# ALIZE-Speaker-Recognition/LIA_RAL

Measured on AMD Instinct MI355X. Metric: Gframe-Gaussian evals/s (UBM EM pass: LLK + full-posterior statistics), higher is better.
Workload: dtype f64; 1 GPU; TrainWorld EM: 2048-Gaussian diag UBM, 60-dim float32 frames, 10000000 frames per GPU resident in HBM, 1 EM iteration per step; gaussians=2048, dim=60, frames_per_gpu=10000000, partitioning=frames sharded per rank, one RCCL all-reduce of 247810 doubles per step

## Files before the change

lia_ral_amd/csrc/devutil.h:

```cpp
#pragma once
#include <hip/hip_runtime.h>
#include <stdint.h>

typedef double d4 __attribute__((ext_vector_type(4)));

#define MFMA_F64(a, b, c) __builtin_amdgcn_mfma_f64_16x16x4f64((a), (b), (c), 0, 0, 0)

#define GMMIV_NEG_BIG (-1.0e300)
#define GMMIV_ZERO_LLK (-745.1332191019412)
#define GMMIV_PAD_LOGIT (-1.0e9)

__device__ __forceinline__ double gexp(double x)
{
    x = fmax(x, -750.0);
    const double n = __builtin_rint(x * 1.4426950408889634074);
    double r = __builtin_fma(n, -6.93147180369123816490e-01, x);
    r = __builtin_fma(n, -1.90821492927058770002e-10, r);
    double p = 1.6059043836821613e-10;
    p = __builtin_fma(p, r, 2.08767569878681e-09);
    p = __builtin_fma(p, r, 2.505210838544172e-08);
    p = __builtin_fma(p, r, 2.755731922398589e-07);
    p = __builtin_fma(p, r, 2.7557319223985893e-06);
    p = __builtin_fma(p, r, 2.48015873015873e-05);
    p = __builtin_fma(p, r, 1.984126984126984e-04);
// ... 153 lines not shown
    GMMIV_ARGMAX_STEP(0x121)
#undef GMMIV_ARGMAX_STEP
    const double v0 = __hiloint2double(__builtin_amdgcn_readlane(__double2hiint(v), 0), __builtin_amdgcn_readlane(__double2loint(v), 0));
    const int c0 = __builtin_amdgcn_readlane(c, 0);
    double wv = v0;
    int wc = c0;
#pragma unroll
    for (int r = 1; r < 4; ++r) {
        const double ov = __hiloint2double(__builtin_amdgcn_readlane(__double2hiint(v), 16 * r), __builtin_amdgcn_readlane(__double2loint(v), 16 * r));
        const int oc = __builtin_amdgcn_readlane(c, 16 * r);
        if (ov > wv || (ov == wv && oc < wc)) { wv = ov; wc = oc; }
    }
    v = wv;
    c = wc;
}

__device__ __forceinline__ double dpp_f64_0x128(double v) { return __hiloint2double(dpp_i32<0x128>(__double2hiint(v)), dpp_i32<0x128>(__double2loint(v))); }
__device__ __forceinline__ double dpp_f64_0x124(double v) { return __hiloint2double(dpp_i32<0x124>(__double2hiint(v)), dpp_i32<0x124>(__double2loint(v))); }
__device__ __forceinline__ double dpp_f64_0x122(double v) { return __hiloint2double(dpp_i32<0x122>(__double2hiint(v)), dpp_i32<0x122>(__double2loint(v))); }
__device__ __forceinline__ double dpp_f64_0x121(double v) { return __hiloint2double(dpp_i32<0x121>(__double2hiint(v)), dpp_i32<0x121>(__double2loint(v))); }
__device__ __forceinline__ double readlane_f64u(double v, int l)
{
    return __hiloint2double(__builtin_amdgcn_readlane(__double2hiint(v), l), __builtin_amdgcn_readlane(__double2loint(v), l));
}
__device__ __forceinline__ double wave_sum_f64_dpp(double v)
{
    v += dpp_f64_0x128(v); v += dpp_f64_0x124(v); v += dpp_f64_0x122(v); v += dpp_f64_0x121(v);
    return (readlane_f64u(v, 0) + readlane_f64u(v, 16)) + (readlane_f64u(v, 32) + readlane_f64u(v, 48));
}
__device__ __forceinline__ double half_sum_f64_dpp(double v, bool hi)
{
    v += dpp_f64_0x128(v); v += dpp_f64_0x124(v); v += dpp_f64_0x122(v); v += dpp_f64_0x121(v);
    const double a = readlane_f64u(v, 0) + readlane_f64u(v, 16), b = readlane_f64u(v, 32) + readlane_f64u(v, 48);
    return hi ? b : a;
}
__device__ __forceinline__ double half_max_f64_dpp(double v, bool hi)
{
    v = fmax(v, dpp_f64_0x128(v)); v = fmax(v, dpp_f64_0x124(v)); v = fmax(v, dpp_f64_0x122(v)); v = fmax(v, dpp_f64_0x121(v));
    const double a = fmax(readlane_f64u(v, 0), readlane_f64u(v, 16)), b = fmax(readlane_f64u(v, 32), readlane_f64u(v, 48));
    return hi ? b : a;
}
__device__ __forceinline__ double half_min_f64_dpp(double v, bool hi)
{
    v = fmin(v, dpp_f64_0x128(v)); v = fmin(v, dpp_f64_0x124(v)); v = fmin(v, dpp_f64_0x122(v)); v = fmin(v, dpp_f64_0x121(v));
    const double a = fmin(readlane_f64u(v, 0), readlane_f64u(v, 16)), b = fmin(readlane_f64u(v, 32), readlane_f64u(v, 48));
    return hi ? b : a;
}
__device__ __forceinline__ double wave_max_f64_dpp(double v)
{
    v = fmax(v, dpp_f64_0x128(v)); v = fmax(v, dpp_f64_0x124(v)); v = fmax(v, dpp_f64_0x122(v)); v = fmax(v, dpp_f64_0x121(v));
    return fmax(fmax(readlane_f64u(v, 0), readlane_f64u(v, 16)), fmax(readlane_f64u(v, 32), readlane_f64u(v, 48)));
}
__device__ __forceinline__ double wave_min_f64_dpp(double v)
{
    v = fmin(v, dpp_f64_0x128(v)); v = fmin(v, dpp_f64_0x124(v)); v = fmin(v, dpp_f64_0x122(v)); v = fmin(v, dpp_f64_0x121(v));
    return fmin(fmin(readlane_f64u(v, 0), readlane_f64u(v, 16)), fmin(readlane_f64u(v, 32), readlane_f64u(v, 48)));
}

__device__ __forceinline__ double shfl_xor_f64(double v, int mask)
{
    int lo = __double2loint(v), hi = __double2hiint(v);
    lo = __shfl_xor(lo, mask, 64);
    hi = __shfl_xor(hi, mask, 64);
    return __hiloint2double(hi, lo);
}

__device__ __forceinline__ double wave_sum_f64(double v)
{
#pragma unroll
    for (int o = 32; o > 0; o >>= 1) v += shfl_xor_f64(v, o);
    return v;
}
__device__ __forceinline__ double wave_max_f64(double v)
{
#pragma unroll
    for (int o = 32; o > 0; o >>= 1) v = fmax(v, shfl_xor_f64(v, o));
    return v;
}

__device__ __forceinline__ int xswz(int t) { return ((t << 1) ^ ((t & 1) << 4)) & 31; }

__device__ __forceinline__ int xrot(int t) { return ((t & 1) << 4) + (((t >> 1) & 7) << 1); }

__device__ __forceinline__ int div_by_magic(unsigned e, unsigned magic) { return magic ? (int)__umulhi(e, magic) : (int)e; }
static inline unsigned gmmiv_div_magic(int D) { return D == 1 ? 0u : (unsigned)((1ULL << 32) / (unsigned)D + 1); }

#define GMMIV_UNUSABLE_BOUND 1e18
#define GMMIV_UNUSABLE_READ_AS 1e10
#ifndef GMMIV_FEAT_SANE_OFF
__device__ __forceinline__ float feat_sane(float v) { return __builtin_fabsf(v) <= (float)GMMIV_UNUSABLE_BOUND ? v : (float)GMMIV_UNUSABLE_READ_AS; }
__device__ __forceinline__ double feat_sane(double v) { return __builtin_fabs(v) <= GMMIV_UNUSABLE_BOUND ? v : GMMIV_UNUSABLE_READ_AS; }
#else
__device__ __forceinline__ float feat_sane(float v) { return v; }
__device__ __forceinline__ double feat_sane(double v) { return v; }
#endif
template <typename T> struct feat_load;
template <> struct feat_load<float> {
    static __device__ __forceinline__ double get(const void *p, long i) { return (double)feat_sane(((const float *)p)[i]); }
    static __device__ __forceinline__ double raw(const void *p, long i) { return (double)((const float *)p)[i]; }
};
template <> struct feat_load<double> {
    static __device__ __forceinline__ double get(const void *p, long i) { return feat_sane(((const double *)p)[i]); }
    static __device__ __forceinline__ double raw(const void *p, long i) { return ((const double *)p)[i]; }
};
```

lia_ral_amd/csrc/gmm_kernels.hip:

```cpp
#include <atomic>
#include "devutil.h"
#include "lds_attr.h"
#include "gmm_kernels.h"

typedef double d2v __attribute__((ext_vector_type(2)));

__global__ void k_gmm_const(int C, int Cp, int D, const double *__restrict__ w,
                            const double *__restrict__ mean, const double *__restrict__ iv,
                            double *__restrict__ a, double *__restrict__ logwcst)
{
    int c = blockIdx.x * blockDim.x + threadIdx.x;
    if (c >= Cp) return;
    if (c >= C) { a[c] = GMMIV_NEG_BIG; logwcst[c] = GMMIV_NEG_BIG; return; }
    double sl = 0.0, sm = 0.0;
    for (int d = 0; d < D; ++d) {
        double v = iv[(size_t)c * D + d], m = mean[(size_t)c * D + d];
        sl += log(v);
        sm += m * m * v;
    }
    double lw = (w[c] > 0.0) ? log(w[c]) : GMMIV_NEG_BIG;
    double lc = lw - 0.5 * D * 1.8378770664093454836 + 0.5 * sl;
    lc = fmax(lc, GMMIV_NEG_BIG);
    logwcst[c] = lc;
    a[c] = fmax(lc - 0.5 * sm, GMMIV_NEG_BIG);
// ... 229 lines not shown
                    gexp_tab_reduce(acc[1][h][r], k1[r], r1);
                    acc[0][h][r] = r0;
                    acc[1][h][r] = r1;
                    const int km = k0[r] > k1[r] ? k0[r] : k1[r];
                    nm[r] = km >> GEXP_TAB_BITS;
                    grow |= nm[r] - E[h][r] >= 64;
                }
                if (__builtin_amdgcn_ballot_w64(grow) != 0) {
#pragma unroll
                    for (int r = 0; r < 4; ++r) {
                        nm[r] = row_max_i32(nm[r]);
                        if (nm[r] - E[h][r] >= 64) {
                            int sh = E[h][r] - nm[r];
                            sh = sh < -2000 ? -2000 : sh;
                            sacc[h][r] = __builtin_ldexp(sacc[h][r], sh);
                            E[h][r] = nm[r];
                        }
                    }
                }
#pragma unroll
                for (int r = 0; r < 4; ++r) {
                    const double e0 = gexp_tab_finish(k0[r], acc[0][h][r], E[h][r], etab);
                    const double e1 = gexp_tab_finish(k1[r], acc[1][h][r], E[h][r], etab);
                    sacc[h][r] += (hit0[r] ? 0.0 : e0) + (hit1[r] ? 0.0 : e1);
                }
            }
            return;
        }
        if (WZ || (MODE == 0 && K1_PLAIN_SHARED)) {
            int nm[2][4], k0[2][4], k1[2][4];
            bool grow = false;
#pragma unroll
            for (int h = 0; h < 2; ++h)
#pragma unroll
                for (int r = 0; r < 4; ++r) {
                    double r0, r1;
                    gexp_tab_reduce(acc[0][h][r], k0[h][r], r0);
                    gexp_tab_reduce(acc[1][h][r], k1[h][r], r1);
                    acc[0][h][r] = r0;
                    acc[1][h][r] = r1;
                    const int km = k0[h][r] > k1[h][r] ? k0[h][r] : k1[h][r];
                    nm[h][r] = km >> GEXP_TAB_BITS;
                    grow |= nm[h][r] - E[h][r] >= 64;
                }
            if (__builtin_amdgcn_ballot_w64(grow) != 0) {
#pragma unroll
                for (int h = 0; h < 2; ++h)
#pragma unroll
                    for (int r = 0; r < 4; ++r) {
                        if (!(K1_ABL & 8)) nm[h][r] = row_max_i32(nm[h][r]);
                        if (nm[h][r] - E[h][r] >= 64) {
                            int sh = E[h][r] - nm[h][r];
                            sh = sh < -2000 ? -2000 : sh;
                            sacc[h][r] = __builtin_ldexp(sacc[h][r], sh);
                            E[h][r] = nm[h][r];
                        }
                    }
            }
#pragma unroll
            for (int h = 0; h < 2; ++h)
#pragma unroll
                for (int r = 0; r < 4; ++r) {
                    const double e0 = gexp_tab_finish(k0[h][r], acc[0][h][r], E[h][r], (K1_ABL & 2) ? etab - (k0[h][r] & (GEXP_TAB_N - 1)) : etab);
                    const double e1 = gexp_tab_finish(k1[h][r], acc[1][h][r], E[h][r], (K1_ABL & 2) ? etab - (k1[h][r] & (GEXP_TAB_N - 1)) : etab);
                    sacc[h][r] += e0 + e1;
                    acc[0][h][r] = e0;
                    acc[1][h][r] = e1;
                }
            if (!WZ) return;
            if (!late) asm volatile("s_waitcnt vmcnt(0)" ::: "memory");
            double *zw = zbuf + ((((size_t)(te * GT)) * nfb + (tb >> 4)) * 64 + lane) * 4;
            if (K1_ABL & 4) {
#pragma unroll
                for (int g = 0; g < GT; ++g)
#pragma unroll
                    for (int h = 0; h < 2; ++h) asm volatile("" ::"v"(acc[g][h]));
                return;
            }
#pragma unroll
            for (int g = 0; g < GT; ++g)
#pragma unroll
                for (int h = 0; h < 2; ++h) __builtin_nontemporal_store(acc[g][h], (d4 *)(zw + ((size_t)g * nfb + h) * 256));
            if (i16 == 0 && !(K1_ABL & 32)) {
                int *ew = eit + (size_t)te * (nfb * 16) + tb + q;
#pragma unroll
                for (int h = 0; h < 2; ++h)
#pragma unroll
                    for (int r = 0; r < 4; ++r) ew[h * 16 + 4 * r] = E[h][r];
            }
            return;
        }
        int nm[2][4];
        bool grow = false;
#pragma unroll
        for (int h = 0; h < 2; ++h)
#pragma unroll
            for (int r = 0; r < 4; ++r) {
                nm[h][r] = gexp_tab_exponent(fmax(acc[0][h][r], acc[1][h][r]));
                grow |= nm[h][r] - E[h][r] >= 64;
            }
        if (__builtin_amdgcn_ballot_w64(grow) != 0) {
#pragma unroll
            for (int h = 0; h < 2; ++h)
#pragma unroll
                for (int r = 0; r < 4; ++r)
                    if (nm[h][r] - E[h][r] >= 64) {
                        int sh = E[h][r] - nm[h][r];
                        sh = sh < -2000 ? -2000 : sh;
                        sacc[h][r] = __builtin_ldexp(sacc[h][r], sh);
                        E[h][r] = nm[h][r];
                    }
        }
        unsigned need = 0;
#pragma unroll
        for (int h = 0; h < 2; ++h)
#pragma unroll
            for (int r = 0; r < 4; ++r) {
                nref[h][r] = nm[h][r] > nref[h][r] ? nm[h][r] : nref[h][r];
                need |= (__builtin_amdgcn_ballot_w64(nm[h][r] > nref[h][r] - 57) != 0 ? 1u : 0u) << (h * 4 + r);
            }
        if (__builtin_popcount(need) > 3) {
#pragma unroll
            for (int h = 0; h < 2; ++h)
#pragma unroll
                for (int r = 0; r < 4; ++r)
                    sacc[h][r] += gexp_tab_scaled(acc[0][h][r], E[h][r], etab) + gexp_tab_scaled(acc[1][h][r], E[h][r], etab);
        } else if (need) {
#pragma unroll
            for (int h = 0; h < 2; ++h)
#pragma unroll
                for (int r = 0; r < 4; ++r)
                    if (need & (1u << (h * 4 + r)))
                        sacc[h][r] += gexp_tab_scaled(acc[0][h][r], E[h][r], etab) + gexp_tab_scaled(acc[1][h][r], E[h][r], etab);
        }
    };
    stage(buf0, 0);
    __syncthreads();
    auto step = [&](int tl, bool staged, bool is_late, bool first) __attribute__((always_inline)) {
        double *cur = (tl & 1) ? buf1 : buf0;
        double *nxt = (tl & 1) ? buf0 : buf1;
        if (staged && (TC || dbg < 2) && !(K1_ABL & 16)) stage(nxt, tl + 1);
        if (!is_late) {
            mfma_phase(cur);
            epi_phase(tl);
        } else {
            if (!first) epi_phase(tl - 1);
            mfma_phase(cur);
        }
        if (WZ) {
            if (is_late) asm volatile("s_waitcnt vmcnt(0)" ::: "memory");
            if (!(K1_ABL & 16)) asm volatile("s_waitcnt lgkmcnt(0)\n\ts_barrier" ::: "memory");
        } else {
            __syncthreads();
        }
    };
    if (!late) {
        for (int tl = 0; tl + 1 < ntiles; ++tl) step(tl, true, false, false);
        if (ntiles > 0) step(ntiles - 1, false, false, false);
    } else {
        if (ntiles > 1) step(0, true, true, true);
        for (int tl = 1; tl + 1 < ntiles; ++tl) step(tl, true, true, false);
        if (ntiles > 0) step(ntiles - 1, false, true, ntiles == 1);
    }
    if (late && ntiles > 0) epi_phase(ntiles - 1);
#pragma unroll
    for (int h = 0; h < 2; ++h)
#pragma unroll
        for (int r = 0; r < 4; ++r) {
            int Em = E[h][r];
#pragma unroll
            for (int o = 1; o < 16; o <<= 1) { const int oe = __shfl_xor(Em, o, 64); Em = oe > Em ? oe : Em; }
// ... 1220 lines not shown
```

lia_ral_amd/csrc/stats_z.hip:

```cpp
#include <atomic>
#include "devutil.h"
#include "lds_attr.h"
#include "gmm_kernels.h"

template <int KS, bool SQ, typename XT, bool PRUNE, int NW = 8, int TPW = 2, int FT = 64, int ZD = 2>
__global__ __launch_bounds__(NW * 64, (TPW == 1 ? 4 : 2)) void k_stats_z(const void *__restrict__ x, long ldx, int D, int C, int nct,
                                                    const double *__restrict__ zbuf, long nfb, const int *__restrict__ eit,
                                                    const double *__restrict__ inv, const int *__restrict__ efin, double scale,
                                                    const long *__restrict__ seg_begin, int nseg, int ngrp,
                                                    double *__restrict__ out0, double *__restrict__ out1, int mode, int accum,
                                                    unsigned magicD, double prune_arg)
{
    constexpr int Dp = 4 * KS;
    constexpr int RL = ((Dp + 2 + 31) / 32) * 32;
    constexpr int JT = RL / 16;
    constexpr int NT = NW * 64;
    constexpr int BPT = FT / 16;
    constexpr int NLD = (FT * Dp + NT - 1) / NT;
    constexpr int RLp = RL + 32;
    constexpr int PF = TPW > 2 ? TPW / 2 : 1;
    extern __shared__ __attribute__((aligned(16))) char smem[];
    double *buf0 = (double *)smem;
    double *buf1 = buf0 + FT * RLp;

    const int b = blockIdx.x;
    const int seg_lo = b & 7;
    const int rest = b >> 3;
    const int grp = rest % ngrp;
    const int seg = (rest / ngrp) * 8 + seg_lo;
    if (seg >= nseg) return;

    const int tid = threadIdx.x, lane = tid & 63, wave = tid >> 6;
    const int i16 = lane & 15, q = lane >> 4;
    const int ct0 = (grp * NW + wave) * TPW;
    const bool active = ct0 < nct;

    const long f0 = seg_begin[seg], f1 = seg_begin[seg + 1];
    const long fa = f0 & ~15L;
    const int nblk = f1 > f0 ? (int)((f1 - fa + 15) >> 4) : 0;
    const int ntiles = (nblk + BPT - 1) / BPT;

    d4 S[TPW][JT], S2[TPW][SQ ? JT : 1];
#pragma unroll
    for (int t = 0; t < TPW; ++t) {
#pragma unroll
        for (int j = 0; j < JT; ++j) S[t][j] = (d4){0, 0, 0, 0};
#pragma unroll
        for (int j = 0; j < (SQ ? JT : 1); ++j) S2[t][j] = (d4){0, 0, 0, 0};
    }

    typedef double d2 __attribute__((ext_vector_type(2)));
    XT stg[NLD];
    double stg_inv = 0.0;
    int stg_ef = 0, stg_e[PF];
    const int npad = FT * (RL - D);
    constexpr bool PLAN_IN_REGS = TPW < 4;
    const bool contig = (ldx == D);
    auto plan_pk = [&](int i) -> unsigned {
        const int e = tid + NT * i;
        const int fr = div_by_magic((unsigned)e, magicD), d = e - fr * D;
        return fr < FT ? ((unsigned)fr << 16) | (unsigned)((fr * RLp + xrot(fr) + d) * 8) : 0xffff0000u;
    };
    auto plan_goff = [&](int i) -> unsigned {
        const int e = tid + NT * i;
        const int fr = div_by_magic((unsigned)e, magicD), d = e - fr * D;
        return fr < FT ? (contig ? (unsigned)e : (unsigned)(fr * (int)ldx + d)) : 0u;
    };
    unsigned pk_r[PLAN_IN_REGS ? NLD : 1], goff_r[PLAN_IN_REGS ? NLD : 1];
    if constexpr (PLAN_IN_REGS) {
#pragma unroll
        for (int i = 0; i < NLD; ++i) { pk_r[i] = plan_pk(i); goff_r[i] = plan_goff(i); }
    }
#define PK(i) (PLAN_IN_REGS ? pk_r[PLAN_IN_REGS ? (i) : 0] : plan_pk(i))
#define GOFF(i) (PLAN_IN_REGS ? goff_r[PLAN_IN_REGS ? (i) : 0] : plan_goff(i))
    double *ftile = buf1 + FT * RLp;
    const int *epair[PF];
#pragma unroll
    for (int p = 0; p < PF; ++p) epair[p] = eit + (size_t)(active ? (ct0 >> 1) + p : 0) * (nfb * 16) + fa;
    const int srow = lane & (FT - 1);
    auto issue_stage = [&](int tl) {
        const long fb = fa + (long)tl * FT;
        const long rem = f1 - fb;
        const unsigned lim = rem >= FT ? (unsigned)FT << 16 : (unsigned)rem << 16;
        const XT *xt = (const XT *)x + fb * ldx;
#pragma unroll
        for (int i = 0; i < NLD; ++i) {
            stg[i] = xt[PK(i) < lim ? GOFF(i) : 0u];
        }
        const long t = fb + srow < f1 ? fb + srow : f1 - 1;
        stg_inv = inv[t];
        stg_ef = efin[t];
#pragma unroll
        for (int p = 0; p < PF; ++p) stg_e[p] = epair[p][(long)tl * FT + srow];
    };
    auto finish_stage = [&](double *dst, int buf, int tl) {
        const long fb = fa + (long)tl * FT;
        const long rem = f1 - fb;
        const unsigned lim = rem >= FT ? (unsigned)FT << 16 : (unsigned)rem << 16;
#pragma unroll
        for (int i = 0; i < NLD; ++i)
        {
            const unsigned pki = PK(i);
            if (pki < ((unsigned)FT << 16)) *(double *)((char *)dst + (pki & 0xffffu)) = pki < lim ? (double)feat_sane(stg[i]) : 0.0;
        }
        if (lane < FT) {
            const long t = fb + lane;
#pragma unroll
            for (int p = 0; p < PF; ++p)
                ftile[((buf * NW + wave) * PF + p) * FT + lane] = (t >= f0 && t < f1) ? __builtin_ldexp(stg_inv * scale, stg_e[p] - stg_ef) : 0.0;
        }
    };
    for (int e = tid; e < 2 * npad; e += NT) {
        double *dst = e < npad ? buf0 : buf1;
        const int ee = e < npad ? e : e - npad;
        const int fr = ee / (RL - D), d = D + (ee - fr * (RL - D));
        dst[fr * RLp + xrot(fr) + d] = (d == Dp) ? 1.0 : 0.0;
    }

    const int offS = q * RLp + ((q & 1) << 4) + ((q >> 1) << 1) + i16;

    const double *zp0 = zbuf + ((((size_t)(active ? ct0 : 0)) * nfb + (fa >> 4)) * 64 + lane) * 4;
    const size_t ztile = (size_t)nfb * 256;
    static_assert((FT / 16) % ZD == 0, "the stream sets must divide the blocks of a tile");
    d2 zs[ZD][TPW][2];
#pragma unroll
    for (int b = 0; b < ZD; ++b)
#pragma unroll
        for (int t = 0; t < TPW; ++t) { zs[b][t][0] = (d2){0, 0}; zs[b][t][1] = zs[b][t][0]; }
    auto issue_z = [&](d2 (&z)[TPW][2], int n) {
#pragma unroll
        for (int t = 0; t < TPW; ++t) {
            const d2 *pz = (const d2 *)(zp0 + (size_t)t * ztile + (size_t)n * 256);
            z[t][0] = __builtin_nontemporal_load(pz);
            z[t][1] = __builtin_nontemporal_load(pz + 1);
        }
    };
    static_assert(TPW == 1 || TPW == 2 || TPW == 4, "operand list of PIN_Z");
#define PIN_Z(z)                                                                                              \
    do {                                                                                                      \
        if constexpr (TPW == 1) asm volatile("" : "+v"(z[0][0]), "+v"(z[0][1]));                             \
        else if constexpr (TPW == 2) asm volatile("" : "+v"(z[0][0]), "+v"(z[0][1]), "+v"(z[1][0]), "+v"(z[1][1])); \
        else asm volatile("" : "+v"(z[0][0]), "+v"(z[0][1]), "+v"(z[1][0]), "+v"(z[1][1]), "+v"(z[TPW / 2][0]),     \
                          "+v"(z[TPW / 2][1]), "+v"(z[TPW - 1][0]), "+v"(z[TPW - 1][1]));                      \
    } while (0)

    if (ntiles > 0) {
        issue_stage(0);
        if (active) {
#pragma unroll
            for (int b = 0; b + 1 < ZD; ++b) issue_z(zs[b], b < nblk ? b : nblk - 1);
        }
        finish_stage(buf0, 0, 0);
#pragma unroll
        for (int b = 0; b + 1 < ZD; ++b) PIN_Z(zs[b]);
    }
    __syncthreads();
    auto tile = [&](int tl, bool full) {
        const double *cur = (tl & 1) ? buf1 : buf0;
        double *nxt = (tl & 1) ? buf0 : buf1;
        const bool staged = full || tl + 1 < ntiles;
        if (staged) issue_stage(tl + 1);
        if (active) {
            const double *pS = cur + offS;
            const double *pF = ftile + ((tl & 1) * NW + wave) * PF * FT + q;
            auto block = [&](int fs, d2 (&zc)[TPW][2], d2 (&zn)[TPW][2]) {
                const int n = tl * BPT + fs;
                if (full) issue_z(zn, (ZD == 2 || n + ZD - 1 < nblk) ? n + ZD - 1 : nblk - 1);
                else if (n + ZD - 1 < nblk) issue_z(zn, n + ZD - 1);
#pragma unroll
                for (int r = 0; r < 4; ++r) {
                    double f[PF];
#pragma unroll
                    for (int p = 0; p < PF; ++p) f[p] = pF[p * FT + fs * 16 + 4 * r];
                    double gm[TPW];
                    bool keep = false;
#pragma unroll
                    for (int t = 0; t < TPW; ++t) { gm[t] = zc[t][r >> 1][r & 1] * f[PF > 1 ? t >> 1 : 0]; keep |= gm[t] > prune_arg; }
                    if (PRUNE && __builtin_amdgcn_ballot_w64(keep) == 0) continue;
#pragma unroll
                    for (int j = 0; j < JT; ++j) {
                        const double bv = pS[(fs * 16 + 4 * r) * RLp + 4 * r + 16 * j];
#pragma unroll
                        for (int t = 0; t < TPW; ++t) S[t][j] = MFMA_F64(gm[t], bv, S[t][j]);
                        if (SQ) {
                            const double b2 = bv * bv;
#pragma unroll
                            for (int t = 0; t < TPW; ++t) S2[t][j] = MFMA_F64(gm[t], b2, S2[t][j]);
                        }
                    }
                }
            };
            const int nb = nblk - tl * BPT;
            block(0, zs[0], zs[ZD - 1]);
            if (full || nb > 1) block(1, zs[1 % ZD], zs[0]);
            if (BPT > 2) {
                if (full || nb > 2) block(2, zs[2 % ZD], zs[1 % ZD]);
                if (full || nb > 3) block(3, zs[3 % ZD], zs[2 % ZD]);
            }
#pragma unroll
            for (int b = 0; b + 1 < ZD; ++b) PIN_Z(zs[b]);
        }
        if (staged) finish_stage(nxt, (tl + 1) & 1, tl + 1);
        __syncthreads();
    };
    for (int tl = 0; tl + 1 < ntiles; ++tl) tile(tl, true);
    if (ntiles > 0) tile(ntiles - 1, false);
#undef PIN_Z
#undef PK
#undef GOFF
    if (!active) return;
#pragma unroll
    for (int t = 0; t < TPW; ++t) {
        const int ct = ct0 + t;
        if (mode == 0) {
            const size_t Cp = (size_t)nct * 16;
            double *o = out0 + (size_t)seg * Cp * (2 * RL);
#pragma unroll
            for (int r = 0; r < 4; ++r) {
                const size_t c = (size_t)ct * 16 + q + 4 * r;
#pragma unroll
                for (int j = 0; j < JT; ++j) {
                    double *o1 = o + c * (2 * RL) + 16 * j + i16;
                    *o1 = (accum ? *o1 : 0.0) + S[t][j][r];
                    if (SQ) { double *o2 = o1 + RL; *o2 = (accum ? *o2 : 0.0) + S2[t][j][r]; }
                }
            }
        } else {
            double *N = out0 + (size_t)seg * C;
            double *F = out1 + (size_t)seg * C * D;
#pragma unroll
            for (int r = 0; r < 4; ++r) {
                const int c = ct * 16 + q + 4 * r;
                if (c >= C) continue;
#pragma unroll
                for (int j = 0; j < JT; ++j) {
                    const int col = 16 * j + i16;
                    if (col < D) F[(size_t)c * D + col] = S[t][j][r];
                    else if (col == Dp) N[c] = S[t][j][r];
                }
            }
        }
    }
}

#define HIPCHK(e)                                                         \
    do {                                                                  \
        hipError_t _e = (e);                                              \
        if (_e != hipSuccess) return (int)_e;                             \
    } while (0)

#define g_stats_z_waves (gmmiv_kopts_cur().z_waves)
#define g_stats_z_tv4 (gmmiv_kopts_cur().z_tv4)
#define g_stats_z_depth_em (gmmiv_kopts_cur().z_depth_em)
#define g_stats_z_depth_tv (gmmiv_kopts_cur().z_depth_tv)
int gmmk_stats_z_groups(int nct) { const int tpg = g_stats_z_waves == 4 ? 8 : 16; return (nct + tpg - 1) / tpg; }
int gmmk_stats_z_wg_per_cu(void) { return g_stats_z_waves == 4 ? 2 : 1; }

template <int KS, bool SQ, typename XT, bool PRUNE, int NW, int TPW, int FT, int ZD = 2>
static int launch_z(hipStream_t st, const void *x, long ldx, int D, int C, int nct, const double *zbuf, long nfb, const int *eit,
                    const double *inv, const int *efin, double scale, const long *seg_begin, int nseg, double *out0, double *out1,
                    int mode, int accum, double prune_thr)
{
    constexpr int RL = ((4 * KS + 2 + 31) / 32) * 32;
    constexpr int PF = TPW > 2 ? TPW / 2 : 1;
    const size_t lds = (size_t)2 * FT * (RL + 32) * sizeof(double) + (size_t)2 * NW * PF * FT * sizeof(double);
    HIPCHK((gmmiv_lds_attr<k_stats_z<KS, SQ, XT, PRUNE, NW, TPW, FT, ZD>>(lds)));
    const int ngrp = (nct + TPW * NW - 1) / (TPW * NW);
    const unsigned grid = (unsigned)(ngrp * 8 * ((nseg + 7) / 8));
    const unsigned magicD = gmmiv_div_magic(D);
    k_stats_z<KS, SQ, XT, PRUNE, NW, TPW, FT, ZD><<<grid, NW * 64, lds, st>>>(x, ldx, D, C, nct, zbuf, nfb, eit, inv, efin, scale, seg_begin, nseg, ngrp,
                                                              out0, out1, mode, accum, magicD, prune_thr);
    return (int)hipGetLastError();
}

#define ZARGS st, x, ldx, D, C, nct, zbuf, nfb, eit, inv, efin, scale, seg_begin, nseg, out0, out1, mode, accum, prune_thr
template <int KS, bool SQ, typename XT>
static int launch_z_p(hipStream_t st, const void *x, long ldx, int D, int C, int nct, const double *zbuf, long nfb, const int *eit,
                      const double *inv, const int *efin, double scale, const long *seg_begin, int nseg, double *out0, double *out1,
                      int mode, int accum, double prune_thr)
{
    if (prune_thr > 0.0) return launch_z<KS, SQ, XT, true, 8, 2, 64>(ZARGS);
    if (g_stats_z_waves == 4) return launch_z<KS, SQ, XT, false, 4, 2, 32>(ZARGS);
    if (g_stats_z_waves == 16) return launch_z<KS, SQ, XT, false, 16, 1, 64>(ZARGS);
    if constexpr (!SQ) {
        if (g_stats_z_depth_tv == 4) return launch_z<KS, SQ, XT, false, 8, 2, 64, 4>(ZARGS);
        if (g_stats_z_tv4 && nct % 4 == 0) return launch_z<KS, SQ, XT, false, 8, 4, 64>(ZARGS);
    } else if (g_stats_z_depth_em == 4) return launch_z<KS, SQ, XT, false, 8, 2, 64, 4>(ZARGS);
    return launch_z<KS, SQ, XT, false, 8, 2, 64>(ZARGS);
}

int gmmk_stats_z(hipStream_t st, int KS, int sq, int x_f64, const void *x, long ldx, int D, int C, int nct, const double *zbuf,
                 long nfb, const int *eit, const double *inv, const int *efin, double scale, const long *seg_begin, int nseg,
                 double *out0, double *out1, int mode, int accum, double prune_thr)
{
    if (nseg <= 0) return 0;
#define CASE(K)                                                                                      \
    case K:                                                                                          \
        if (sq) return x_f64 ? launch_z_p<K, true, double>(ZARGS) : launch_z_p<K, true, float>(ZARGS); \
        return x_f64 ? launch_z_p<K, false, double>(ZARGS) : launch_z_p<K, false, float>(ZARGS);
    switch (KS) {
        CASE(4) CASE(8) CASE(15)
    }
#undef CASE
    return -1;
}
```

lia_ral_amd/csrc/topc_z.hip:

```cpp
#include "devutil.h"
#include "gmm_kernels.h"

typedef double d2 __attribute__((ext_vector_type(2)));

template <typename XT>
__global__ __launch_bounds__(256, 2) void k_topc_from_z(const void *__restrict__ x, long n, long ldx, int D, int C, int nct,
                                                        const double *__restrict__ zbuf, long nfb, const int *__restrict__ eit,
                                                        const int *__restrict__ efin, const double *__restrict__ mean,
                                                        const double *__restrict__ iv, const double *__restrict__ lwc,
                                                        const double *__restrict__ w, int ctop, int complete, double lo, double hi,
                                                        int *__restrict__ idx_out, double *__restrict__ lk_out,
                                                        double *__restrict__ nontop_lk, double *__restrict__ nontop_llk,
                                                        double *__restrict__ nontop_w, double *__restrict__ llk_out, int *__restrict__ flag)
{
    __shared__ double xs[8][64 + 1];
    __shared__ int ord[4][64];
    __shared__ __attribute__((aligned(16))) double lmx[4][64];
    __shared__ double thx[4];
    const int tid = threadIdx.x, lane = tid & 63, wave = tid >> 6, i16 = lane & 15, qq = lane >> 4;
    const long fb = blockIdx.x >> 1;
    const int half = blockIdx.x & 1, q0 = wave;
    for (int e = tid; e < 8 * D; e += 256) {
        const int lf = e / D, d = e - lf * D;
        const long t = fb * 16 + (lf >> 1) + 4 * (2 * half + (lf & 1));
        xs[lf][d] = t < n ? feat_load<XT>::get(x, t * ldx + d) : 0.0;
    }
    long tj[2];
    int ef[2];
#pragma unroll
    for (int j = 0; j < 2; ++j) {
        tj[j] = fb * 16 + q0 + 4 * (2 * half + j);
        ef[j] = tj[j] < n ? efin[tj[j]] : 0;
    }
    double val[2][32];
#pragma unroll
    for (int h = 0; h < 2; ++h) {
        d2 e2[16];
        int e0[16], e1[16];
#pragma unroll
        for (int mm = 0; mm < 16; ++mm) {
            const int ct = 4 * (16 * h + mm) + qq, cc = ct < nct ? ct : nct - 1;
            e2[mm] = *(const d2 *)(zbuf + (((size_t)cc * nfb + fb) * 64 + 16 * q0 + i16) * 4 + 2 * half);
            const int *ep = eit + (size_t)(cc >> 1) * (nfb * 16) + fb * 16 + q0 + 8 * half;
            e0[mm] = ep[0];
            e1[mm] = ep[4];
        }
        asm volatile("" ::: "memory");
#pragma unroll
        for (int mm = 0; mm < 16; ++mm) {
            const int m = 16 * h + mm, ct = 4 * m + qq;
            const double a0 = __builtin_ldexp(e2[mm][0], e0[mm] - ef[0]), a1 = __builtin_ldexp(e2[mm][1], e1[mm] - ef[1]);
            val[0][m] = ct < nct ? a0 : -1.0;
            val[1][m] = ct < nct ? a1 : -1.0;
        }
    }
    __syncthreads();

    const double NINF = -__builtin_inf();
    const int K = ctop + 4 < C ? ctop + 4 : C;
#pragma unroll
    for (int j = 0; j < 2; ++j) {
        const long t = tj[j];
        if (t >= n) continue;
        const int lf = 2 * wave + j;
        double lm;
        {
            double t16[16];
#pragma unroll
            for (int i = 0; i < 16; ++i) t16[i] = fmax(val[j][i], val[j][i + 16]);
#pragma unroll
            for (int i = 0; i < 8; ++i) t16[i] = fmax(t16[i], t16[i + 8]);
#pragma unroll
            for (int i = 0; i < 4; ++i) t16[i] = fmax(t16[i], t16[i + 4]);
            lm = fmax(fmax(t16[0], t16[2]), fmax(t16[1], t16[3]));
        }
        lmx[wave][lane] = lm;
        __builtin_amdgcn_fence(__ATOMIC_RELEASE, "wavefront");
        __builtin_amdgcn_wave_barrier();
        __builtin_amdgcn_fence(__ATOMIC_ACQUIRE, "wavefront");
        int lrank = 0;
#pragma unroll
        for (int i = 0; i < 64; ++i) {
            const double o = lmx[wave][i];
            lrank += (o > lm || (o == lm && i < lane)) ? 1 : 0;
        }
        if (lrank == K - 1) thx[wave] = lm;
        __builtin_amdgcn_fence(__ATOMIC_RELEASE, "wavefront");
        __builtin_amdgcn_wave_barrier();
        __builtin_amdgcn_fence(__ATOMIC_ACQUIRE, "wavefront");
        double theta = thx[wave];
        __builtin_amdgcn_wave_barrier();
        if (!(theta > 0.0)) theta = 4.9e-324;
        int nc = 0;
#pragma unroll
        for (int m = 0; m < 32; ++m) {
            const bool hit = val[j][m] >= theta;
            const unsigned long long mask = __builtin_amdgcn_ballot_w64(hit);
            if (mask) {
                if (hit) {
                    const int pos = nc + __builtin_popcountll(mask & ((1ull << lane) - 1ull));
                    if (pos < 64) ord[wave][pos] = 16 * (4 * m + qq) + i16;
                }
                nc += __builtin_popcountll(mask);
            }
        }
        __builtin_amdgcn_fence(__ATOMIC_RELEASE, "wavefront");
        __builtin_amdgcn_wave_barrier();
        __builtin_amdgcn_fence(__ATOMIC_ACQUIRE, "wavefront");
        if (nc > 64) { if (lane == 0) atomicExch(flag, 1); continue; }
        if (nc < (ctop < C ? ctop : C)) { if (lane == 0) atomicExch(flag, 1); continue; }
        const int ci = lane < nc ? ord[wave][lane] : 0x7fffffff;
        __builtin_amdgcn_wave_barrier();
        const double vnext = theta;
        const bool cand = lane < nc && ci < C;
        double zc = NINF;
        if (cand) {
            const double *mu = mean + (size_t)ci * D, *vi = iv + (size_t)ci * D;
            double acc = 0.0;
            int d = 0;
            for (; d + 8 <= D; d += 8) {
                double m8[8], v8[8];
#pragma unroll
                for (int u = 0; u < 8; ++u) { m8[u] = mu[d + u]; v8[u] = vi[d + u]; }
#pragma unroll
                for (int u = 0; u < 8; ++u) {
                    const double dx = xs[lf][d + u] - m8[u];
                    acc = __builtin_fma(dx * dx, v8[u], acc);
                }
// ... 664 lines not shown
    const d2 *mu = (const d2 *)(cl.mean + (size_t)cc * D), *vi = (const d2 *)(cl.iv + (size_t)cc * D);
    const int np = D >> 1;
    double acc = 0.0;
    for (int p0 = 0; p0 < np; p0 += 16) {
        d2 m[4], v[4];
        double x0[4], x1[4];
#pragma unroll
        for (int u = 0; u < 4; ++u) {
            const int p = p0 + sub + 4 * u, pc = p < np ? p : np - 1;
            m[u] = mu[pc];
            v[u] = vi[pc];
            x0[u] = feat_load<XT>::get(x, t * ldx + 2 * pc);
            x1[u] = feat_load<XT>::get(x, t * ldx + 2 * pc + 1);
        }
#pragma unroll
        for (int u = 0; u < 4; ++u) {
            const bool ok = p0 + sub + 4 * u < np;
            const double dx0 = x0[u] - m[u][0], dx1 = x1[u] - m[u][1];
            const double a1 = __builtin_fma(dx1 * dx1, v[u][1], __builtin_fma(dx0 * dx0, v[u][0], acc));
            acc = ok ? a1 : acc;
        }
    }
    acc += __hiloint2double(dpp_i32<0xB1>(__double2hiint(acc)), dpp_i32<0xB1>(__double2loint(acc)));
    acc += __hiloint2double(dpp_i32<0x4E>(__double2hiint(acc)), dpp_i32<0x4E>(__double2loint(acc)));
    const double z = live ? __builtin_fma(-0.5, acc, cl.lwc[cc]) : NINF;
    const double r = (complete && nontop_llk) ? nontop_llk[t] : NINF;
    const double M = wave_max_f64_dpp(fmax(z, r));
    const double s0 = wave_sum_f64_dpp((live && sub == 0) ? gexp(z - M) : 0.0);
    if (lane == 0) {
        const double s = r > NINF ? s0 + gexp(r - M) : s0;
        llk_out[(size_t)blockIdx.y * T + t] = fmin(fmax(M + log(s), lo), hi);
    }
}
int gmmk_topc_use4_multi(hipStream_t st, int x_f64, const void *x, long T, long ldx, int D, const void *clients, int n_clients, int ctop,
                         const int *idx, const double *nllk, int complete, double lo, double hi, double *llk)
{
    if (T <= 0 || n_clients <= 0) return 0;
    if (ctop > 16 || D % 2 != 0 || n_clients > 65535) return -1;
    const dim3 grid((unsigned)((T + 3) / 4), (unsigned)n_clients);
    if (x_f64) k_topc_use4_multi<double><<<grid, 256, 0, st>>>(x, T, ldx, D, (const TopcClient *)clients, ctop, idx, nllk, complete, lo, hi, llk);
    else k_topc_use4_multi<float><<<grid, 256, 0, st>>>(x, T, ldx, D, (const TopcClient *)clients, ctop, idx, nllk, complete, lo, hi, llk);
    return (int)hipGetLastError();
}

int gmmk_topc_use16(hipStream_t st, int x_f64, const void *x, long T, long ldx, int D, const double *mean, const double *iv,
                    const double *lwc, int C, int ctop, const int *idx, const double *nllk, int complete, double lo, double hi, double *llk,
                    int four)
{
    if (T <= 0) return 0;
    if (ctop > 16 || D % 2 != 0) return -1;
    if (four == 4) {
        const unsigned grid4 = (unsigned)((T + 3) / 4);
        if (x_f64) k_topc_use4<double><<<grid4, 256, 0, st>>>(x, T, ldx, D, mean, iv, lwc, C, ctop, idx, nllk, complete, lo, hi, llk);
        else k_topc_use4<float><<<grid4, 256, 0, st>>>(x, T, ldx, D, mean, iv, lwc, C, ctop, idx, nllk, complete, lo, hi, llk);
        return (int)hipGetLastError();
    }
    const unsigned grid = (unsigned)((T + 15) / 16);
    const size_t lds = (size_t)16 * (D + 1) * sizeof(double);
    if (x_f64) k_topc_use16<double><<<grid, 256, lds, st>>>(x, T, ldx, D, mean, iv, lwc, C, ctop, idx, nllk, complete, lo, hi, llk);
    else k_topc_use16<float><<<grid, 256, lds, st>>>(x, T, ldx, D, mean, iv, lwc, C, ctop, idx, nllk, complete, lo, hi, llk);
    return (int)hipGetLastError();
}

__global__ __launch_bounds__(256) void k_post_from_z(long n, int C, int nct, const double *__restrict__ zbuf, long nfb,
                                                     const int *__restrict__ eit, const double *__restrict__ inv,
                                                     const int *__restrict__ efin, double *__restrict__ gamma)
{
    const int lane = threadIdx.x & 63, wave = threadIdx.x >> 6, i16 = lane & 15, q = lane >> 4;
    const long fb = blockIdx.x;
    double fs[4];
    int ef[4];
    long tr[4];
#pragma unroll
    for (int r = 0; r < 4; ++r) {
        tr[r] = fb * 16 + q + 4 * r;
        const long tc = tr[r] < n ? tr[r] : n - 1;
        fs[r] = inv[tc];
        ef[r] = efin[tc];
    }
    for (int ct = blockIdx.y * 4 + wave; ct < nct; ct += gridDim.y * 4) {
        const d2 *pz = (const d2 *)(zbuf + (((size_t)ct * nfb + fb) * 64 + lane) * 4);
        const d2 a = __builtin_nontemporal_load(pz), b = __builtin_nontemporal_load(pz + 1);
        const double e[4] = {a[0], a[1], b[0], b[1]};
        const int *ep = eit + (size_t)(ct >> 1) * (nfb * 16) + fb * 16 + q;
        const int c = 16 * ct + i16;
#pragma unroll
        for (int r = 0; r < 4; ++r)
            if (tr[r] < n && c < C) gamma[(size_t)tr[r] * C + c] = __builtin_ldexp(e[r] * fs[r], ep[4 * r] - ef[r]);
    }
}

int gmmk_post_from_z(hipStream_t st, long n, int C, int nct, const double *zbuf, long nfb, const int *eit, const double *inv,
                     const int *efin, double *gamma)
{
    if (n <= 0) return 0;
    const unsigned gy = nct >= 32 ? 8 : 1;
    k_post_from_z<<<dim3((unsigned)((n + 15) / 16), gy), 256, 0, st>>>(n, C, nct, zbuf, nfb, eit, inv, efin, gamma);
    return (int)hipGetLastError();
}
```

Measured before the change: 125.7 Gframe-Gaussian/s.

## Permute exponent table for vector stores and stage x,x² pairs in LDS

The per-tile exponent table is reordered so each lane group writes its four exponents with one 16-byte vector store instead of four scattered scalar stores. Every reader (stats, top-C, posterior) is updated to index through the new slot mapping. For the main squared-stats configuration, the stats kernel now stores each feature together with its square as an adjacent pair in LDS. This removes the per-MFMA multiply and lets one 16-byte LDS load feed both products, at the cost of doubling the LDS row size, which may lower occupancy.

```diff
diff --git a/lia_ral_amd/csrc/devutil.h b/lia_ral_amd/csrc/devutil.h
--- a/lia_ral_amd/csrc/devutil.h
+++ b/lia_ral_amd/csrc/devutil.h
@@ -259,6 +259,8 @@
 
 __device__ __forceinline__ int xrot(int t) { return ((t & 1) << 4) + (((t >> 1) & 7) << 1); }
 
+__device__ __forceinline__ int eit_slot(int t) { return (t & ~15) | ((t & 3) << 2) | ((t >> 2) & 3); }
+
 __device__ __forceinline__ int div_by_magic(unsigned e, unsigned magic) { return magic ? (int)__umulhi(e, magic) : (int)e; }
 static inline unsigned gmmiv_div_magic(int D) { return D == 1 ? 0u : (unsigned)((1ULL << 32) / (unsigned)D + 1); }
 
diff --git a/lia_ral_amd/csrc/gmm_kernels.hip b/lia_ral_amd/csrc/gmm_kernels.hip
--- a/lia_ral_amd/csrc/gmm_kernels.hip
+++ b/lia_ral_amd/csrc/gmm_kernels.hip
@@ -335,11 +335,10 @@
 #pragma unroll
                 for (int h = 0; h < 2; ++h) __builtin_nontemporal_store(acc[g][h], (d4 *)(zw + ((size_t)g * nfb + h) * 256));
             if (i16 == 0 && !(K1_ABL & 32)) {
-                int *ew = eit + (size_t)te * (nfb * 16) + tb + q;
-#pragma unroll
-                for (int h = 0; h < 2; ++h)
-#pragma unroll
-                    for (int r = 0; r < 4; ++r) ew[h * 16 + 4 * r] = E[h][r];
+                typedef int i4 __attribute__((ext_vector_type(4)));
+                int *ew = eit + (size_t)te * (nfb * 16) + tb + 4 * q;
+#pragma unroll
+                for (int h = 0; h < 2; ++h) *(i4 *)(ew + h * 16) = (i4){E[h][0], E[h][1], E[h][2], E[h][3]};
             }
             return;
         }
diff --git a/lia_ral_amd/csrc/stats_z.hip b/lia_ral_amd/csrc/stats_z.hip
--- a/lia_ral_amd/csrc/stats_z.hip
+++ b/lia_ral_amd/csrc/stats_z.hip
@@ -2,6 +2,9 @@
 #include "devutil.h"
 #include "lds_attr.h"
 #include "gmm_kernels.h"
+
+static constexpr bool z_x2_in_lds(bool SQ, bool PRUNE, int NW, int TPW, int FT) { return SQ && !PRUNE && NW == 8 && TPW == 2 && FT == 64; }
+static constexpr int z_row_len(int RL, bool x2) { return x2 ? 2 * RL : RL + 32; }
 
 template <int KS, bool SQ, typename XT, bool PRUNE, int NW = 8, int TPW = 2, int FT = 64, int ZD = 2>
 __global__ __launch_bounds__(NW * 64, (TPW == 1 ? 4 : 2)) void k_stats_z(const void *__restrict__ x, long ldx, int D, int C, int nct,
@@ -17,7 +20,8 @@
     constexpr int NT = NW * 64;
     constexpr int BPT = FT / 16;
     constexpr int NLD = (FT * Dp + NT - 1) / NT;
-    constexpr int RLp = RL + 32;
+    constexpr bool X2 = z_x2_in_lds(SQ, PRUNE, NW, TPW, FT);
+    constexpr int RLp = z_row_len(RL, X2);
     constexpr int PF = TPW > 2 ? TPW / 2 : 1;
     extern __shared__ __attribute__((aligned(16))) char smem[];
     double *buf0 = (double *)smem;
@@ -59,6 +63,7 @@
     auto plan_pk = [&](int i) -> unsigned {
         const int e = tid + NT * i;
         const int fr = div_by_magic((unsigned)e, magicD), d = e - fr * D;
+        if constexpr (X2) return fr < FT ? ((unsigned)fr << 16) | (unsigned)(fr * RLp + 2 * d) : 0xffff0000u;
         return fr < FT ? ((unsigned)fr << 16) | (unsigned)((fr * RLp + xrot(fr) + d) * 8) : 0xffff0000u;
     };
     auto plan_goff = [&](int i) -> unsigned {
@@ -91,7 +96,7 @@
         stg_inv = inv[t];
         stg_ef = efin[t];
 #pragma unroll
-        for (int p = 0; p < PF; ++p) stg_e[p] = epair[p][(long)tl * FT + srow];
+        for (int p = 0; p < PF; ++p) stg_e[p] = epair[p][(long)tl * FT + eit_slot(srow)];
     };
     auto finish_stage = [&](double *dst, int buf, int tl) {
         const long fb = fa + (long)tl * FT;
@@ -101,7 +106,12 @@
         for (int i = 0; i < NLD; ++i)
         {
             const unsigned pki = PK(i);
-            if (pki < ((unsigned)FT << 16)) *(double *)((char *)dst + (pki & 0xffffu)) = pki < lim ? (double)feat_sane(stg[i]) : 0.0;
+            if constexpr (X2) {
+                if (pki < ((unsigned)FT << 16)) {
+                    const double v = pki < lim ? (double)feat_sane(stg[i]) : 0.0;
+                    *(d2 *)(dst + (pki & 0xffffu)) = (d2){v, v * v};
+                }
+            } else if (pki < ((unsigned)FT << 16)) *(double *)((char *)dst + (pki & 0xffffu)) = pki < lim ? (double)feat_sane(stg[i]) : 0.0;
         }
         if (lane < FT) {
             const long t = fb + lane;
@@ -114,10 +124,11 @@
         double *dst = e < npad ? buf0 : buf1;
         const int ee = e < npad ? e : e - npad;
         const int fr = ee / (RL - D), d = D + (ee - fr * (RL - D));
-        dst[fr * RLp + xrot(fr) + d] = (d == Dp) ? 1.0 : 0.0;
-    }
-
-    const int offS = q * RLp + ((q & 1) << 4) + ((q >> 1) << 1) + i16;
+        if constexpr (X2) *(d2 *)(dst + fr * RLp + 2 * d) = (d == Dp) ? (d2){1.0, 1.0} : (d2){0.0, 0.0};
+        else dst[fr * RLp + xrot(fr) + d] = (d == Dp) ? 1.0 : 0.0;
+    }
+
+    const int offS = X2 ? q * RLp + 2 * i16 : q * RLp + ((q & 1) << 4) + ((q >> 1) << 1) + i16;
 
     const double *zp0 = zbuf + ((((size_t)(active ? ct0 : 0)) * nfb + (fa >> 4)) * 64 + lane) * 4;
     const size_t ztile = (size_t)nfb * 256;
@@ -179,11 +190,15 @@
                     if (PRUNE && __builtin_amdgcn_ballot_w64(keep) == 0) continue;
 #pragma unroll
                     for (int j = 0; j < JT; ++j) {
-                        const double bv = pS[(fs * 16 + 4 * r) * RLp + 4 * r + 16 * j];
+                        const double *pb = pS + (fs * 16 + 4 * r) * RLp + (X2 ? 32 * j : 4 * r + 16 * j);
+                        d2 bb;
+                        if constexpr (X2) bb = *(const d2 *)pb;
+                        else bb[0] = pb[0];
+                        const double bv = bb[0];
 #pragma unroll
                         for (int t = 0; t < TPW; ++t) S[t][j] = MFMA_F64(gm[t], bv, S[t][j]);
                         if (SQ) {
-                            const double b2 = bv * bv;
+                            const double b2 = X2 ? bb[1] : bv * bv;
 #pragma unroll
                             for (int t = 0; t < TPW; ++t) S2[t][j] = MFMA_F64(gm[t], b2, S2[t][j]);
                         }
@@ -263,7 +278,7 @@
 {
     constexpr int RL = ((4 * KS + 2 + 31) / 32) * 32;
     constexpr int PF = TPW > 2 ? TPW / 2 : 1;
-    const size_t lds = (size_t)2 * FT * (RL + 32) * sizeof(double) + (size_t)2 * NW * PF * FT * sizeof(double);
+    const size_t lds = (size_t)2 * FT * z_row_len(RL, z_x2_in_lds(SQ, PRUNE, NW, TPW, FT)) * sizeof(double) + (size_t)2 * NW * PF * FT * sizeof(double);
     HIPCHK((gmmiv_lds_attr<k_stats_z<KS, SQ, XT, PRUNE, NW, TPW, FT, ZD>>(lds)));
     const int ngrp = (nct + TPW * NW - 1) / (TPW * NW);
     const unsigned grid = (unsigned)(ngrp * 8 * ((nseg + 7) / 8));
diff --git a/lia_ral_amd/csrc/topc_z.hip b/lia_ral_amd/csrc/topc_z.hip
--- a/lia_ral_amd/csrc/topc_z.hip
+++ b/lia_ral_amd/csrc/topc_z.hip
@@ -41,9 +41,9 @@
         for (int mm = 0; mm < 16; ++mm) {
             const int ct = 4 * (16 * h + mm) + qq, cc = ct < nct ? ct : nct - 1;
             e2[mm] = *(const d2 *)(zbuf + (((size_t)cc * nfb + fb) * 64 + 16 * q0 + i16) * 4 + 2 * half);
-            const int *ep = eit + (size_t)(cc >> 1) * (nfb * 16) + fb * 16 + q0 + 8 * half;
+            const int *ep = eit + (size_t)(cc >> 1) * (nfb * 16) + fb * 16 + eit_slot(q0 + 8 * half);
             e0[mm] = ep[0];
-            e1[mm] = ep[4];
+            e1[mm] = ep[1];
         }
         asm volatile("" ::: "memory");
 #pragma unroll
@@ -874,11 +874,11 @@
         const d2 *pz = (const d2 *)(zbuf + (((size_t)ct * nfb + fb) * 64 + lane) * 4);
         const d2 a = __builtin_nontemporal_load(pz), b = __builtin_nontemporal_load(pz + 1);
         const double e[4] = {a[0], a[1], b[0], b[1]};
-        const int *ep = eit + (size_t)(ct >> 1) * (nfb * 16) + fb * 16 + q;
+        const int *ep = eit + (size_t)(ct >> 1) * (nfb * 16) + fb * 16 + eit_slot(q);
         const int c = 16 * ct + i16;
 #pragma unroll
         for (int r = 0; r < 4; ++r)
-            if (tr[r] < n && c < C) gamma[(size_t)tr[r] * C + c] = __builtin_ldexp(e[r] * fs[r], ep[4 * r] - ef[r]);
+            if (tr[r] < n && c < C) gamma[(size_t)tr[r] * C + c] = __builtin_ldexp(e[r] * fs[r], ep[r] - ef[r]);
     }
 }
 
```

Result: faster. 127.8 Gframe-Gaussian/s (median of 6 runs) (+1.7%).
